# librosa/librosa

Measured on AMD Instinct MI355X. Metric: STFT+mel frames/sec (n_fft=2048 hop=512), higher is better.
Workload: dtype f32

## Files before the change

### librosa_amd/csrc/lra_fft.h

```cpp
#pragma once

#include <cmath>

#include "lra_common.h"

namespace lra {

template <int LOGM_, int LOGR_, class T_, int NTMIN_ = 256, int MINW_ = 0, bool HOIST_ = true, bool REV_ = false, int PLAN_ = 0> struct FftCfg {
    using real = T_;
    using cplx = cx<T_>;
    static constexpr int LOGM = LOGM_;
    static constexpr int M = 1 << LOGM_;
    static constexpr int N = 2 * M;
    static constexpr int LOGR = LOGR_ < LOGM_ ? LOGR_ : LOGM_;
    static constexpr int R = 1 << LOGR;
    static constexpr int TF = M / R;
    static constexpr int NT = TF > NTMIN_ ? TF : NTMIN_;
    static constexpr int FPB = NT / TF;
    static constexpr int P = (LOGM + LOGR - 1) / LOGR;
    static constexpr bool REV = REV_;
    static constexpr int PLAN = PLAN_;
    static constexpr int logr(int p) {
        if (PLAN_ == 1 && REV_) return p == 0 ? LOGM - (P - 1) * LOGR : LOGR;
        if (PLAN_ == 1) return (p + 1) * LOGR <= LOGM ? LOGR : LOGM - p * LOGR;
        return LOGM / P + ((REV_ ? p >= P - LOGM % P : p < LOGM % P) ? 1 : 0);
    }
    static constexpr int logs(int p) {
        int s = 0;
        for (int q = 0; q < p; ++q) s += logr(q);
        return s;
    }
    static constexpr int tw_off(int p) {
        int o = 0;
        for (int q = 1; q < p; ++q) o += ((1 << logr(q)) - 1) << logs(q);
        return o;
    }
    static constexpr int TW_TOTAL = tw_off(P) > 0 ? tw_off(P) : 1;
    static constexpr int treg_off(int p) {
        int o = 0;
        for (int q = 1; q < p; ++q) o += (R >> logr(q)) * logr(q);
        return o;
    }
    static constexpr int TREG_TOTAL = treg_off(P) > 0 ? treg_off(P) : 1;
    static constexpr int PADSHIFT = logr(0);
    static constexpr int FRAME_ELEMS = M + (M >> PADSHIFT) + 1;
    static constexpr int FRAME_BYTES = ((FRAME_ELEMS * (int)sizeof(cplx) + 15) / 16) * 16;
    static constexpr int phys(int i) { return i + (i >> PADSHIFT); }
    static constexpr int MIN_WAVES = MINW_ > 0 ? MINW_ : 2;
    static constexpr bool HOIST = HOIST_;
    template <int NT2> using with_nt = FftCfg<LOGM_, LOGR_, T_, NT2, MINW_, HOIST_, REV_, PLAN_>;
    static constexpr bool WAVE_SYNC = TF <= 64;
};

template <class T> LRA_HD cx<T> mul_w16(cx<T> a, int idx) {
    const T h = (T)0.70710678118654752440;
    const T c1 = (T)0.92387953251128675613, s1 = (T)0.38268343236508977173;
    switch (idx) {
        case 0: return a;
        case 4: return cmul_mi(a);
        case 2: return mk<T>((a.x + a.y) * h, (a.y - a.x) * h);
        case 6: return mk<T>((a.y - a.x) * h, -(a.x + a.y) * h);
        case 1: return mk<T>(a.x * c1 + a.y * s1, a.y * c1 - a.x * s1);
        case 3: return mk<T>(a.x * s1 + a.y * c1, a.y * s1 - a.x * c1);
        case 5: return mk<T>(a.y * c1 - a.x * s1, -(a.x * c1 + a.y * s1));
        default:  return mk<T>(a.y * s1 - a.x * c1, -(a.x * s1 + a.y * c1));
    }
}

template <int idx, class T> LRA_HD void bfly_w16(cx<T> e, cx<T> o, cx<T>& p, cx<T>& m) {
    const T h = (T)0.70710678118654752440;
    const T c1 = (T)0.92387953251128675613, s1 = (T)0.38268343236508977173;
    if constexpr (idx == 0) {
        p = cadd(e, o);
        m = csub(e, o);
    } else if constexpr (idx == 4) {
        p = add_mi(e, o);
        m = sub_mi(e, o);
    } else if constexpr (idx == 2) {
        const cx<T> u = add_mi(o, o);
        p = axpy(h, u, e);
        m = axpy(-h, u, e);
    } else if constexpr (idx == 6) {
        const cx<T> u = add_mi(o, o);
        p = axpy_mi(h, u, e);
        m = axpy_pi(h, u, e);
    } else if constexpr (idx == 1 || idx == 3) {
        const T c = idx == 1 ? c1 : s1, s = idx == 1 ? s1 : c1;
        p = axpy_mi(s, o, axpy(c, o, e));
        m = axpy_pi(s, o, axpy(-c, o, e));
    } else {
        const T c = idx == 5 ? c1 : s1, s = idx == 5 ? s1 : c1;
        p = axpy_mi(c, o, axpy(-s, o, e));
        m = axpy_pi(c, o, axpy(s, o, e));
    }
}

template <int r, class T> struct Dft {
    template <int k> static LRA_HD void stage(cx<T>* v, const cx<T>* e, const cx<T>* o) {
        if constexpr (k < r / 2) {
            bfly_w16<k * (16 / r), T>(e[k], o[k], v[k], v[k + r / 2]);
            stage<k + 1>(v, e, o);
        }
    }
    static LRA_HD void run(cx<T>* v) {
        cx<T> e[r / 2], o[r / 2];
        LRA_UNROLL
        for (int k = 0; k < r / 2; ++k) { e[k] = v[2 * k]; o[k] = v[2 * k + 1]; }
        Dft<r / 2, T>::run(e);
        Dft<r / 2, T>::run(o);
        stage<0>(v, e, o);
    }
};
template <class T> struct Dft<1, T> {
    static LRA_HD void run(cx<T>*) {}
};
template <class T> struct Dft<2, T> {
    static LRA_HD void run(cx<T>* v) {
        const cx<T> a = v[0], b = v[1];
        v[0] = cadd(a, b);
        v[1] = csub(a, b);
    }
};

template <class Cfg> constexpr int pstride(int c) { return c + (c >> Cfg::PADSHIFT); }
template <class Cfg> constexpr bool affine_tf() { return Cfg::TF % (1 << Cfg::PADSHIFT) == 0; }

template <class Cfg, int p> LRA_HD void pass_read(typename Cfg::cplx* v, Lds fr, int tf) {
    using C = typename Cfg::cplx;
    constexpr int lr = Cfg::logr(p), r = 1 << lr, nb = Cfg::R >> lr, sin = Cfg::M >> lr, Q = 1 << Cfg::PADSHIFT;
    if constexpr (affine_tf<Cfg>() && sin % Q == 0) {
        const int base = Cfg::phys(tf) * (int)sizeof(C);
        LRA_UNROLL
        for (int i = 0; i < nb; ++i) {
            LRA_UNROLL
            for (int j = 0; j < r; ++j) v[i * r + j] = lds_ld<C>(fr, base + (i * pstride<Cfg>(Cfg::TF) + j * pstride<Cfg>(sin)) * (int)sizeof(C));
        }
    } else {
        LRA_UNROLL
        for (int i = 0; i < nb; ++i) {
            const int b = tf + i * Cfg::TF;
            LRA_UNROLL
            for (int j = 0; j < r; ++j) v[i * r + j] = lds_ld<C>(fr, Cfg::phys(b + j * sin) * (int)sizeof(C));
        }
    }
}

template <class Cfg, int p> LRA_HD void pass_twiddle_dft(typename Cfg::cplx* v, int tf, const typename Cfg::cplx* __restrict__ tw) {
    using T = typename Cfg::real;
    constexpr int lr = Cfg::logr(p), r = 1 << lr, nb = Cfg::R >> lr, s = 1 << Cfg::logs(p);
    LRA_UNROLL
    for (int i = 0; i < nb; ++i) {
        const int b = tf + i * Cfg::TF;
        if (p > 0) {
            const int k = b & (s - 1);
            typename Cfg::cplx q[r];
            LRA_UNROLL
            for (int j = 1; j < r; ++j) q[j] = cmul_p(v[i * r + j], tw[Cfg::tw_off(p) + (j - 1) * s + k]);
            LRA_UNROLL
            for (int j = 1; j < r; ++j) v[i * r + j] = cmul_f(v[i * r + j], tw[Cfg::tw_off(p) + (j - 1) * s + k], q[j]);
        }
        Dft<r, T>::run(v + i * r);
    }
}

constexpr int popcount_c(int j) { int c = 0; for (; j; j >>= 1) c += j & 1; return c; }
constexpr int msb_c(int j) { int m = 0; for (int t = 0; t < 16; ++t) if ((j >> t) & 1) m = t; return m; }

template <class Cfg, int p> LRA_HD void pass_twiddle_dft_reg(typename Cfg::cplx* v, const typename Cfg::cplx* treg) {
    using T = typename Cfg::real;
    using C = typename Cfg::cplx;
    constexpr int lr = Cfg::logr(p), r = 1 << lr, nb = Cfg::R >> lr;
    LRA_UNROLL
    for (int i = 0; i < nb; ++i) {
        if (p > 0) {
            C w[r], q[r];
            LRA_UNROLL
            for (int j = 1; j < r; ++j)
                if (popcount_c(j) == 1) w[j] = treg[Cfg::treg_off(p) + i * lr + msb_c(j)];
            LRA_UNROLL
            for (int level = 2; level <= lr; ++level) {
                LRA_UNROLL
                for (int j = 1; j < r; ++j)
                    if (popcount_c(j) == level) q[j] = cmul_p(w[j - (1 << msb_c(j))], treg[Cfg::treg_off(p) + i * lr + msb_c(j)]);
                LRA_UNROLL
                for (int j = 1; j < r; ++j)
                    if (popcount_c(j) == level) w[j] = cmul_f(w[j - (1 << msb_c(j))], treg[Cfg::treg_off(p) + i * lr + msb_c(j)], q[j]);
            }
            LRA_UNROLL
            for (int j = 1; j < r; ++j) q[j] = cmul_p(v[i * r + j], w[j]);
            LRA_UNROLL
            for (int j = 1; j < r; ++j) v[i * r + j] = cmul_f(v[i * r + j], w[j], q[j]);
        }
        Dft<r, T>::run(v + i * r);
    }
}

template <class Cfg, int p> LRA_HD void load_pass_twiddles(typename Cfg::cplx* treg, int tf, const typename Cfg::cplx* __restrict__ tw) {
    constexpr int lr = Cfg::logr(p), nb = Cfg::R >> lr, s = 1 << Cfg::logs(p);
    LRA_UNROLL
    for (int i = 0; i < nb; ++i) {
        const int k = (tf + i * Cfg::TF) & (s - 1);
        LRA_UNROLL
        for (int t = 0; t < lr; ++t) treg[Cfg::treg_off(p) + i * lr + t] = tw[Cfg::tw_off(p) + ((1 << t) - 1) * s + k];
    }
}

template <class Cfg, int p> LRA_HD void pass_write(const typename Cfg::cplx* v, Lds fr, int tf) {
    using C = typename Cfg::cplx;
    constexpr int lr = Cfg::logr(p), r = 1 << lr, nb = Cfg::R >> lr, s = 1 << Cfg::logs(p);
    constexpr bool last = p == Cfg::P - 1;
    if constexpr (affine_tf<Cfg>() && p == 0) {
        const int base = tf * (r + 1) * (int)sizeof(C);
        LRA_UNROLL
        for (int i = 0; i < nb; ++i) {
            LRA_UNROLL
            for (int j = 0; j < r; ++j) lds_st<C>(fr, base + (i * Cfg::TF * (r + 1) + j) * (int)sizeof(C), v[i * r + j]);
        }
    } else if constexpr (affine_tf<Cfg>() && p > 0 && (last || Cfg::TF % s == 0)) {
        int base;
        if (last) {
            base = Cfg::phys(tf) * (int)sizeof(C);
        } else {
            const int k = tf & (s - 1);
            base = Cfg::phys(((tf - k) << lr) + k) * (int)sizeof(C);
        }
        constexpr int istep = last ? pstride<Cfg>(Cfg::TF) : pstride<Cfg>(Cfg::TF << lr);
        LRA_UNROLL
        for (int i = 0; i < nb; ++i) {
            LRA_UNROLL
            for (int j = 0; j < r; ++j) lds_st<C>(fr, base + (i * istep + j * pstride<Cfg>(s)) * (int)sizeof(C), v[i * r + j]);
        }
    } else {
        LRA_UNROLL
        for (int i = 0; i < nb; ++i) {
            const int b = tf + i * Cfg::TF;
            const int k = b & (s - 1);
            const int base = ((b - k) << lr) + k;
            LRA_UNROLL
            for (int j = 0; j < r; ++j) lds_st<C>(fr, Cfg::phys(base + j * s) * (int)sizeof(C), v[i * r + j]);
        }
    }
}

template <class Cfg> LRA_HD int last_pass_pos(int tf, int i, int j) {
    constexpr int p = Cfg::P - 1, s = 1 << Cfg::logs(p);
    return (tf + i * Cfg::TF) + j * s;
}

template <class Cfg> inline void build_pass_twiddles(typename Cfg::cplx* out) {
    const double two_pi = 6.283185307179586476925286766559;
    for (int p = 1; p < Cfg::P; ++p) {
        const int r = 1 << Cfg::logr(p), s = 1 << Cfg::logs(p);
        for (int j = 1; j < r; ++j)
            for (int k = 0; k < s; ++k) {
                const double ang = -two_pi * (double)k * (double)j / ((double)s * (double)r);
                out[Cfg::tw_off(p) + (j - 1) * s + k] = mk<typename Cfg::real>((typename Cfg::real)std::cos(ang), (typename Cfg::real)std::sin(ang));
            }
    }
}
template <class Cfg> constexpr int split_tw_count() { return Cfg::M + 1; }
template <class Cfg> inline void build_split_twiddles(typename Cfg::cplx* out) {
    const double two_pi = 6.283185307179586476925286766559;
    for (int k = 0; k <= Cfg::M; ++k) {
        const double ang = -two_pi * (double)k / (double)Cfg::N;
        out[k] = mk<typename Cfg::real>((typename Cfg::real)std::cos(ang), (typename Cfg::real)std::sin(ang));
    }
}

}
```

### librosa_amd/csrc/lra_kernels2.h

```cpp
#pragma once

#include "lra_kernels.h"

namespace lra {

template <class Cfg> constexpr bool v2_cfg_ok() {
    constexpr int pl = Cfg::P - 1;
    return Cfg::P >= 2 && Cfg::R == 16 && Cfg::HOIST && sizeof(typename Cfg::real) == 4 && affine_tf<Cfg>() && (Cfg::R >> Cfg::logr(pl)) == 2 &&
           2 * Cfg::TF == (Cfg::M >> Cfg::logr(pl)) && (Cfg::M >> Cfg::logr(pl)) % (1 << Cfg::PADSHIFT) == 0;
}
template <class Cfg> constexpr bool v2_hd_ok(int hd) { return (hd == 1 || hd == 2 || hd == 4 || hd == 8) && (1 << Cfg::logr(0)) % hd == 0; }
template <class Cfg> LRA_HD int v2_hop_divisor(int hop) {
    for (int hd = 1; hd <= 8; hd *= 2)
        if (hop * hd == Cfg::N && v2_hd_ok<Cfg>(hd)) return hd;
    return 0;
}

constexpr int kV2PrioA = 3, kV2PrioS = 2, kV2PrioB = 0, kV2PrioB3 = 1;
constexpr int kV2PrioCA = 3, kV2PrioCS = 2;
constexpr int kV2PrioPA = 3, kV2PrioPS = 2;
template <int P> LRA_HD void v2_setprio() { lra_setprio<P>(); }

template <class Cfg, int HD> struct Regs2 {
    using C = typename Cfg::cplx;
// ... 55 lines not shown
    using RG = Regs2<Cfg, HD>;
    if (next >= a.n_frames) return;
    const T* __restrict__ yb = a.y + (long long)clip * a.y_stride;
    const long long p0 = (long long)next * a.hop;
    const long long g0 = p0 + (Cfg::N - a.hop) - a.pad;
    if (LRA_LIKELY(g0 >= 0 && g0 + a.hop <= a.n)) {
        const T* __restrict__ src = yb + (p0 - a.pad) + 2 * tf;
        if (LRA_LIKELY((reinterpret_cast<size_t>(src) & (2 * sizeof(T) - 1)) == 0)) {
            LRA_UNROLL
            for (int n = 0; n < RG::NEW; ++n) {
                const int e = RG::elem_of_new(n);
                rg.pf[n] = *reinterpret_cast<const C*>(src + 2 * ((e / RG::r0) * Cfg::TF + (e % RG::r0) * RG::sin0));
            }
        } else {
            LRA_UNROLL
            for (int n = 0; n < RG::NEW; ++n) {
                const int e = RG::elem_of_new(n);
                const T* __restrict__ s2 = src + 2 * ((e / RG::r0) * Cfg::TF + (e % RG::r0) * RG::sin0);
                rg.pf[n] = mk<T>(s2[0], s2[1]);
            }
        }
    } else {
        LRA_UNROLL
        for (int n = 0; n < RG::NEW; ++n) {
            const long long p = p0 + 2 * RG::q_of(tf, RG::elem_of_new(n));
            rg.pf[n] = mk<T>(fetch_sample<T>(yb, p, a.pad, a.n, a.pad_mode), fetch_sample<T>(yb, p + 1, a.pad, a.n, a.pad_mode));
        }
    }
}

template <class Cfg, int HD> LRA_HD void v2_fill(const StftArgs<typename Cfg::real>& a, int clip, int frame, int tf, Regs2<Cfg, HD>& rg) {
    using T = typename Cfg::real;
    using RG = Regs2<Cfg, HD>;
    const T* __restrict__ yb = a.y + (long long)clip * a.y_stride;
    const long long p0 = (long long)frame * a.hop;
    LRA_UNROLL
    for (int e = 0; e < Cfg::R; ++e) {
        const long long p = p0 + 2 * RG::q_of(tf, e);
        const bool live = frame < a.n_frames;
        rg.raw[e] = live ? mk<T>(fetch_sample<T>(yb, p, a.pad, a.n, a.pad_mode), fetch_sample<T>(yb, p + 1, a.pad, a.n, a.pad_mode)) : mk<T>((T)0, (T)0);
    }
}

template <class Cfg, int HD> LRA_HD void v2_shift(Regs2<Cfg, HD>& rg) {
    using RG = Regs2<Cfg, HD>;
    LRA_UNROLL
    for (int i = 0; i < RG::nb0; ++i) {
        LRA_UNROLL
        for (int j = 0; j < RG::r0; ++j) rg.raw[i * RG::r0 + j] = j + RG::SJ < RG::r0 ? rg.raw[i * RG::r0 + j + RG::SJ] : rg.pf[i * RG::SJ + (j + RG::SJ - RG::r0)];
    }
}

template <class Cfg, int HD> LRA_HD void v2_window_rotating_ref(int it, Regs2<Cfg, HD>& rg) {
    using T = typename Cfg::real;
    using RG = Regs2<Cfg, HD>;
    constexpr int r0 = RG::r0, nb0 = RG::nb0, SJ = RG::SJ;
    const int rot = it & (HD - 1);
    for (int i = 0; i < nb0; ++i) {
        if (it > 0)
            for (int m = 0; m < SJ; ++m) rg.raw[i * r0 + (SJ * ((rot + HD - 1) % HD) + m) % r0] = rg.pf[i * SJ + m];
        for (int j = 0; j < r0; ++j) {
            const typename Cfg::cplx x = rg.raw[i * r0 + (j + SJ * rot) % r0], w = rg.win2[i * r0 + j];
            rg.v[i * r0 + j] = mk<T>(x.x * w.x, x.y * w.y);
        }
    }
}
template <class Cfg, int HD> constexpr bool v2_rotate_asm_ok() {
    return HD == 4 && Regs2<Cfg, HD>::r0 == 16 && Regs2<Cfg, HD>::nb0 == 1 && sizeof(typename Cfg::real) == 4;
}
#if defined(LRA_PK_ASM)
__device__ __forceinline__ void v2_rot_class(pk::f2& p0, pk::f2& p1, pk::f2& p2, pk::f2& p3, pk::f2 pf, pk::f2 w0, pk::f2 w1, pk::f2 w2, pk::f2 w3, pk::f2& v0, pk::f2& v1,
                                              pk::f2& v2, pk::f2& v3, int rot, int ins) {
    asm("s_cmp_lg_u32 %13, 0\n\t"
        "s_cbranch_scc1 .Lrot1_%=\n\t"
        "s_cmp_eq_u32 %14, 0\n\t"
        "s_cbranch_scc1 .Lrot0_%=\n\t"
        "v_mov_b64 %7, %8\n"
        ".Lrot0_%=:\n\t"
        "v_pk_mul_f32 %0, %4, %9\n\t"
        "v_pk_mul_f32 %1, %5, %10\n\t"
        "v_pk_mul_f32 %2, %6, %11\n\t"
        "v_pk_mul_f32 %3, %7, %12\n\t"
        "s_branch .Lrotend_%=\n"
        ".Lrot1_%=:\n\t"
        "s_cmp_lg_u32 %13, 1\n\t"
        "s_cbranch_scc1 .Lrot2_%=\n\t"
        "v_pk_mul_f32 %0, %5, %9\n\t"
        "v_pk_mul_f32 %1, %6, %10\n\t"
        "v_pk_mul_f32 %2, %7, %11\n\t"
        "v_pk_mul_f32 %3, %8, %12\n\t"
        "v_mov_b64 %4, %8\n\t"
        "s_branch .Lrotend_%=\n"
        ".Lrot2_%=:\n\t"
        "s_cmp_lg_u32 %13, 2\n\t"
        "s_cbranch_scc1 .Lrot3_%=\n\t"
        "v_pk_mul_f32 %0, %6, %9\n\t"
        "v_pk_mul_f32 %1, %7, %10\n\t"
        "v_pk_mul_f32 %2, %4, %11\n\t"
        "v_pk_mul_f32 %3, %8, %12\n\t"
        "v_mov_b64 %5, %8\n\t"
        "s_branch .Lrotend_%=\n"
        ".Lrot3_%=:\n\t"
        "v_pk_mul_f32 %0, %7, %9\n\t"
        "v_pk_mul_f32 %1, %4, %10\n\t"
        "v_pk_mul_f32 %2, %5, %11\n\t"
        "v_pk_mul_f32 %3, %8, %12\n\t"
        "v_mov_b64 %6, %8\n"
        ".Lrotend_%=:\n\t"
        "s_nop 0"
        : "=&v"(v0), "=&v"(v1), "=&v"(v2), "=&v"(v3), "+v"(p0), "+v"(p1), "+v"(p2), "+v"(p3)
        : "v"(pf), "v"(w0), "v"(w1), "v"(w2), "v"(w3), "s"(rot), "s"(ins)
        : "scc");
}
#endif
template <class Cfg, int HD> LRA_HD void v2_window_rotating(int it, Regs2<Cfg, HD>& rg) {
#if defined(LRA_PK_ASM)
    if constexpr (v2_rotate_asm_ok<Cfg, HD>()) {
        const int rot = it & 3, ins = it;
        pk::f2 p[16], o[16];
        LRA_UNROLL
        for (int e = 0; e < 16; ++e) p[e] = pk::v(rg.raw[e]);
        LRA_UNROLL
        for (int c = 0; c < 4; ++c)
            v2_rot_class(p[c], p[c + 4], p[c + 8], p[c + 12], pk::v(rg.pf[c]), pk::v(rg.win2[c]), pk::v(rg.win2[c + 4]), pk::v(rg.win2[c + 8]), pk::v(rg.win2[c + 12]), o[c],
                         o[c + 4], o[c + 8], o[c + 12], rot, ins);
        LRA_UNROLL
        for (int e = 0; e < 16; ++e) { rg.raw[e] = pk::c(p[e]); rg.v[e] = pk::c(o[e]); }
        return;
    }
#endif
    v2_window_rotating_ref<Cfg, HD>(it, rg);
}
template <class Cfg, int HD> LRA_HD void v2_pass0_dft(int tf, Regs2<Cfg, HD>& rg, Lds fr) {
    using T = typename Cfg::real;
    constexpr int r0 = Regs2<Cfg, HD>::r0, nb0 = Regs2<Cfg, HD>::nb0;
    LRA_UNROLL
    for (int i = 0; i < nb0; ++i) Dft<r0, T>::run(rg.v + i * r0);
    pass_write<Cfg, 0>(rg.v, fr, tf);
}

template <class Cfg, int HD> LRA_HD void v2_pass0(bool live, int tf, Regs2<Cfg, HD>& rg, Lds fr) {
    using T = typename Cfg::real;
    constexpr int r0 = Regs2<Cfg, HD>::r0, nb0 = Regs2<Cfg, HD>::nb0;
    (void)live;
    LRA_UNROLL
    for (int e = 0; e < Cfg::R; ++e) rg.v[e] = mk<T>(rg.raw[e].x * rg.win2[e].x, rg.raw[e].y * rg.win2[e].y);
    LRA_UNROLL
    for (int i = 0; i < nb0; ++i) Dft<r0, T>::run(rg.v + i * r0);
    pass_write<Cfg, 0>(rg.v, fr, tf);
}

template <class Cfg, int HD> LRA_HD void v2_last_read(Regs2<Cfg, HD>& rg, Lds fr, int tf) {
    using C = typename Cfg::cplx;
    constexpr int p = Cfg::P - 1, lr = Cfg::logr(p), r = 1 << lr, sin = Cfg::M >> lr;
    const int bA = Cfg::phys(tf) * (int)sizeof(C);
    const int bB = Cfg::phys(v2_mirror_bfly<Cfg>(tf)) * (int)sizeof(C);
    LRA_UNROLL
    for (int j = 0; j < r; ++j) {
        rg.v[j] = lds_ld<C>(fr, bA + j * pstride<Cfg>(sin) * (int)sizeof(C));
        rg.v[r + j] = lds_ld<C>(fr, bB + j * pstride<Cfg>(sin) * (int)sizeof(C));
    }
}


template <class T> struct alignas(16) V4 {
    T a, b, c, d;
};
template <class Cfg> constexpr bool v2_pw_swz() { return (2 * Cfg::TF) % 128 == 0; }
template <bool SWZ> LRA_HD int v2_pw_index_t(int k) {
    if (SWZ) return (k >> 3) * 8 + ((((k >> 2) ^ (k >> 7)) & 1) << 2) + (k & 3);
    return (k >> 3) * 12 + (k & 7);
}
template <class Cfg> LRA_HD int v2_pw_index(int k) { return v2_pw_index_t<v2_pw_swz<Cfg>()>(k); }
template <class Cfg> constexpr int v2_pw_bytes() { return (v2_pw_swz<Cfg>() ? Cfg::M + 8 : (Cfg::M >> 3) * 12 + 4) * (int)sizeof(typename Cfg::real); }

template <class Cfg> LRA_HD void v2_pw_addr_xor(Lds stage, int tf, int tfh, bool l0, int (&ak)[2][2], int (&am)[2][2]) {
    using T = typename Cfg::real;
    constexpr int p = Cfg::P - 1, r = 1 << Cfg::logr(p), s = 2 * Cfg::TF, M = Cfg::M, SZ = (int)sizeof(T);
    static_assert(v2_pw_swz<Cfg>() && SZ == 4 && s == 128, "bit 4 of the byte address swaps the halves of a run, bit 7 of the bin selects");
    constexpr int LOW = M - (r - 1) * s;
    ak[0][0] = lds_addr(stage, tf * SZ);
    ak[1][0] = lds_addr(stage, tfh * SZ);
    am[1][1] = lds_addr(stage, (LOW - tfh) * SZ);
    LRA_UNROLL
    for (int f = 0; f < 2; ++f) ak[f][1] = ak[f][0] ^ 16;
    am[1][0] = am[1][1] ^ 16;
    am[0][0] = l0 ? lds_addr(stage, LOW * SZ) : am[1][0];
    am[0][1] = am[0][0] ^ 16;
}

template <class Cfg, int HD, int MODE, int PM, bool PIN = true>
LRA_HD void v2_last_split_store(const StftArgs<typename Cfg::real>& a, int clip, int frame, bool valid, int tf, Regs2<Cfg, HD>& rg, Lds stage) {
    using T = typename Cfg::real;
    using C = typename Cfg::cplx;
    constexpr int p = Cfg::P - 1, r = 1 << Cfg::logr(p), s = 2 * Cfg::TF, M = Cfg::M;
    static_assert(r * s == M, "last pass: r butterfly outputs s apart");
    pass_twiddle_dft_reg<Cfg, p>(rg.v, rg.treg);
    const C* A = rg.v;
    const C* B = rg.v + r;
    const bool l0 = tf == 0;
    const LaneMask l0m = lane_mask(l0);
    const int tfh = v2_tf_hi<Cfg>(tf);
    const long long row = ((long long)clip * a.n_frames + frame) * a.row_pitch;
    C* __restrict__ const D = MODE == OUT_COMPLEX ? a.D + row : nullptr;
    T* __restrict__ const S = MODE == OUT_POWER ? a.S + row : nullptr;
    int pwk[2][2] = {{0, 0}, {0, 0}}, pwm[2][2] = {{0, 0}, {0, 0}};
    constexpr bool AXOR = MODE == OUT_MELR && !PIN && v2_pw_swz<Cfg>();
    constexpr bool POW2 = MODE == OUT_MELR && PM == POW_TWO;
    int ak[2][2] = {{0, 0}, {0, 0}}, am[2][2] = {{0, 0}, {0, 0}};
    if constexpr (AXOR) v2_pw_addr_xor<Cfg>(stage, tf, tfh, l0, ak, am);
    if (MODE == OUT_MELR && !AXOR) {
        LRA_UNROLL
        for (int par = 0; par < 2; ++par) {
            pwk[0][par] = v2_pw_index<Cfg>(tf + par * s) * (int)sizeof(T);
            pwk[1][par] = v2_pw_index<Cfg>(tfh + par * s) * (int)sizeof(T);
            pwm[0][par] = v2_pw_index<Cfg>(M - tf - par * s) * (int)sizeof(T);
            pwm[1][par] = v2_pw_index<Cfg>(M - tfh - par * s) * (int)sizeof(T);
            if (PIN) { LRA_KEEP(pwk[0][par]); LRA_KEEP(pwk[1][par]); LRA_KEEP(pwm[0][par]); LRA_KEEP(pwm[1][par]); }
        }
    }
    LRA_UNROLL
    for (int q = 0; q < r; ++q) {
        const C zk = q >= r / 2 ? sel_mask(l0m, l0, B[q - r / 2], A[q]) : A[q];
        C zm;
        if (q == 0) zm = B[r - 1];
        else if (q < r / 2) zm = sel_mask(l0m, l0, A[r - q], B[r - 1 - q]);
        else zm = sel_mask(l0m, l0, B[3 * r / 2 - 1 - q], B[r - 1 - q]);
        C xk = mk<T>((T)0, (T)0), xm = xk;
        C pp = xk;
        if constexpr (POW2) pp = split_pair_pow2<T>(zk, zm, rg.twr[q]);
        else split_pair<T>(zk, zm, rg.twr[q], xk, xm);
        if (q == 0) {
            const C z0 = A[0];
            const C dc = mk<T>((T)2 * (z0.x + z0.y), (T)0), ny = mk<T>((T)2 * (z0.x - z0.y), (T)0);
            if constexpr (POW2) {
                pp = mk<T>(sel_mask(l0m, l0, dc.x * dc.x, pp.x), sel_mask(l0m, l0, ny.x * ny.x, pp.y));
            } else {
                xk = sel_mask(l0m, l0, dc, xk);
                xm = sel_mask(l0m, l0, ny, xm);
            }
            if (LRA_UNLIKELY(l0 && valid && a.nonfinite_flag && !(std::fabs(dc.x) <= std::numeric_limits<T>::max()))) LRA_ATOMIC_OR(a.nonfinite_flag, 1u);
        }
        const int k = (q < r / 2 ? tf : tfh) + q * s;
        if (MODE == OUT_MELR) {
            const T vk = POW2 ? pp.x : spec_power<T, PM>(xk, a.power), vm = POW2 ? pp.y : spec_power<T, PM>(xm, a.power);
            if constexpr (AXOR) {
                lds_st_addr<T>(stage, ak[q < r / 2 ? 0 : 1][q & 1] + ((q & 1) * s + (q >> 1) * 2 * s) * (int)sizeof(T), vk);
                lds_st_addr<T>(stage, am[q < r / 2 ? 0 : 1][q & 1] + ((1 - (q & 1)) * s + (r / 2 - 1 - (q >> 1)) * 2 * s) * (int)sizeof(T), vm);
            } else if (v2_pw_swz<Cfg>()) {
                lds_st<T>(stage, pwk[q < r / 2 ? 0 : 1][q & 1] + (q >> 1) * 2 * s * (int)sizeof(T), vk);
                lds_st<T>(stage, pwm[q < r / 2 ? 0 : 1][q & 1] - (q >> 1) * 2 * s * (int)sizeof(T), vm);
            } else {
                lds_st<T>(stage, pwk[q < r / 2 ? 0 : 1][0] + 24 * q * (s / 16) * (int)sizeof(T), vk);
                lds_st<T>(stage, pwm[q < r / 2 ? 0 : 1][0] - 24 * q * (s / 16) * (int)sizeof(T), vm);
            }
        } else if (MODE == OUT_COMPLEX) {
            if (valid) { stream_store(&D[k], xk); stream_store(&D[M - k], xm); }
        } else {
            const T pk = spec_power<T, PM>(xk, a.power), pm = spec_power<T, PM>(xm, a.power);
            if (valid) { S[k] = pk; S[M - k] = pm; }
        }
    }
    const C zmid = A[r / 2];
    const C xmid = mk<T>((T)2 * zmid.x, (T)-2 * zmid.y);
    if (MODE == OUT_MELR) {
        if (l0) lds_st<T>(stage, v2_pw_index<Cfg>(M / 2) * (int)sizeof(T), spec_power<T, PM>(xmid, a.power));
    } else if (l0 && valid) {
        if (MODE == OUT_COMPLEX) D[M / 2] = xmid;
        else S[M / 2] = spec_power<T, PM>(xmid, a.power);
    }
}


template <class Cfg, int HD> LRA_HD void v2_mel_runs_read(Regs2<Cfg, HD>& rg, Lds pwr, int tf) {
    using T = typename Cfg::real;
    constexpr int BPL = Cfg::R / 2;
    static_assert(BPL == 8, "runs of 8 bins");
    LRA_UNROLL
    for (int run = 0; run < 2; ++run) {
        const int first = 8 * (run * Cfg::TF + tf);
        const V4<T> lo = lds_ld<V4<T>>(pwr, v2_pw_index<Cfg>(first) * (int)sizeof(T)), hi = lds_ld<V4<T>>(pwr, v2_pw_index<Cfg>(first + 4) * (int)sizeof(T));
        T* d = rg.pw + run * BPL;
        d[0] = lo.a; d[1] = lo.b; d[2] = lo.c; d[3] = lo.d; d[4] = hi.a; d[5] = hi.b; d[6] = hi.c; d[7] = hi.d;
    }
    rg.pw_extra = lds_ld<T>(pwr, (tf == 0 ? v2_pw_index<Cfg>(Cfg::M) : 0) * (int)sizeof(T));
}

template <class Cfg, int HD> LRA_HD void v2_mel_weights_read(Regs2<Cfg, HD>& rg, Lds sh, int tf) {
    using T = typename Cfg::real;
    constexpr int BPL = Cfg::R / 2, TF = Cfg::TF;
    LRA_UNROLL
    for (int run = 0; run < 2; ++run) {
        LRA_UNROLL
        for (int j = 0; j < BPL; j += 2) {
            const V4<T> w2 = lds_ld<V4<T>>(sh, ((BPL + 2) * (run * TF + tf) + j) * 2 * (int)sizeof(T));
            rg.v[run * BPL + j] = mk<T>(w2.a, w2.b);
            rg.v[run * BPL + j + 1] = mk<T>(w2.c, w2.d);
        }
    }
}

template <class Cfg, int HD> LRA_HD void v2_mel_accumulate(const StftArgs<typename Cfg::real>& a, int tf, Regs2<Cfg, HD>& rg, Lds rs, Lds sh) {
    using T = typename Cfg::real;
    using C = typename Cfg::cplx;
    constexpr int BPL = Cfg::R / 2, TF = Cfg::TF;
    const C* w = rg.v;
    LRA_UNROLL
    for (int run = 0; run < 2; ++run) {
        C acc = mk<T>((T)0, (T)0);
        LRA_UNROLL
        for (int j = 0; j < BPL; ++j) {
            const int jj = run * BPL + j;
            const T p = rg.pw[jj], keep = rg.keep[jj];
// ... 331 lines not shown
```

### librosa_amd/csrc/lra_kernels_pc.h

```cpp
#pragma once

#include "lra_kernels2.h"

namespace lra {

constexpr int kPcPrioPA = 3, kPcPrioPS = 2, kPcPrioCA = 0, kPcPrioCB = 1;
constexpr int kPcSpinLimit = 1 << 22;

template <class Cfg> struct PcLayout {
    using T = typename Cfg::real;
    static constexpr int NP = 2;
    static constexpr int NT = (NP + 1) * Cfg::TF;
    static constexpr int FRAME = Cfg::FRAME_BYTES;
    static constexpr int PW = (v2_pw_bytes<Cfg>() + 15) / 16 * 16;
    static constexpr int RS = ((Cfg::R * (Cfg::TF + kMelRsPitchExtra) + 2) * 2 * (int)sizeof(T) + 15) / 16 * 16;
    static constexpr int frame_off(int s) { return s * FRAME; }
    static constexpr int pw_off(int s) { return NP * FRAME + s * PW; }
    static constexpr int rs_off() { return NP * (FRAME + PW); }
    static constexpr int flags_off() { return rs_off() + RS; }
    static constexpr int ready_off(int s) { return flags_off() + 4 * s; }
    static constexpr int consumed_off(int s) { return flags_off() + 4 * (NP + s); }
    static constexpr int BYTES = flags_off() + 16;
};

// ... 23 lines not shown
    C w[Cfg::R];
    C wq;
    T keep[Cfg::R];
    T pw[Cfg::R], pw_extra;
    int mad[NB][2 * PH];
    int pwa[4], pwx;
    T* row[NB];
    int ph[NP][NB];
    PcTileV mt[NP];
};
template <class Cfg> LRA_HD bool pc_tile_uniform(const StftArgs<typename Cfg::real>& a) { return (a.n_frames & 3) == 0 && Cfg::TF >= 64; }
#ifdef LRA_HOSTSIM
LRA_HD int pc_mad_addr(Lds wg, int ad) { return ad; }
LRA_HD cx<float> pc_pair_ld(Lds wg, int addr) { return lds_ld<cx<float>>(wg, addr); }
#else
__device__ __forceinline__ int pc_mad_addr(Lds wg, int ad) {
    int addr = (int)(unsigned int)(size_t)(__attribute__((address_space(3))) char*)(wg.base + ad);
    asm volatile("" : "+v"(addr));
    return addr;
}
__device__ __forceinline__ cx<float> pc_pair_ld(Lds, int addr) {
    typedef float f2v __attribute__((ext_vector_type(2)));
    const f2v t = *(const volatile __attribute__((address_space(3))) f2v*)(size_t)(unsigned int)addr;
    return __builtin_bit_cast(cx<float>, t);
}
#endif
template <class T, int MT> LRA_HD void pc_tile_band(const PcTileV& t, int b, T (&out)[MT]) {
    LRA_UNROLL
    for (int k = 0; k < MT; ++k) out[k] = t[MT * b + k];
}

#ifdef LRA_HOSTSIM
LRA_HD int pc_flag_load(Lds l, int off) { return lds_ld<int>(l, off); }
LRA_HD void pc_flag_store(Lds l, int off, int v) { lds_st<int>(l, off, v); }
LRA_HD void pc_wait(Lds, int, int, unsigned int*) {}
LRA_HD void pc_fence() {}
#else
__device__ __forceinline__ void pc_fence() {
    __builtin_amdgcn_fence(__ATOMIC_RELEASE, "wavefront");
    __builtin_amdgcn_wave_barrier();
    __builtin_amdgcn_fence(__ATOMIC_ACQUIRE, "wavefront");
}
__device__ __forceinline__ int pc_flag_load(Lds l, int off) { return *(const volatile __attribute__((address_space(3))) int*)(l.base + off); }
__device__ __forceinline__ void pc_flag_store(Lds l, int off, int v) { *(volatile __attribute__((address_space(3))) int*)(l.base + off) = v; }
__device__ __forceinline__ void pc_wait(Lds l, int off, int want, unsigned int* sticky) {
    int spins = 0;
    while (true) {
        const int v = LRA_UNIFORM(pc_flag_load(l, off));
        if (LRA_LIKELY(v >= want)) break;
        if (LRA_UNLIKELY(++spins > kPcSpinLimit)) {
            if (sticky && (threadIdx.x & 63) == 0) atomicOr(sticky, 2u);
            break;
        }
        __builtin_amdgcn_s_sleep(2);
    }
    pc_fence();
}
__device__ __forceinline__ void pc_wait_ready(Lds l, int off, int want, unsigned int* sticky) {
    if (LRA_UNLIKELY(LRA_UNIFORM(pc_flag_load(l, off)) < want)) pc_wait(l, off, want, sticky);
    else pc_fence();
}
#endif

template <class Cfg, int HD> LRA_HD void pc_producer_prologue(const StftArgs<typename Cfg::real>& a, int clip, int frame0, int tf, Regs2<Cfg, HD>& rg) {
    using T = typename Cfg::real;
    if constexpr (Cfg::PLAN == 1) v3_hoist<Cfg, HD>(rg, tf, a.win, a.tw, a.twr);
    else v2_hoist<Cfg, HD>(rg, tf, a.win, a.tw, a.twr);
    v2_fill<Cfg, HD>(a, clip, frame0, tf, rg);
    if constexpr (v2_rotate_asm_ok<Cfg, HD>()) {
        LRA_UNROLL
        for (int e = 0; e < Cfg::R; ++e) { LRA_KEEP(rg.raw[e].x); LRA_KEEP(rg.raw[e].y); }
    }
    LRA_UNROLL
    for (int e = 0; e < Regs2<Cfg, HD>::NEW; ++e) rg.pf[e] = mk<T>((T)0, (T)0);
}
template <class Cfg, int HD> LRA_HD void pc_producer_pass0(const StftArgs<typename Cfg::real>& a, int clip, int frame, int it, bool more, int tf, Regs2<Cfg, HD>& rg, Lds fr) {
    if (v2_rotate_asm_ok<Cfg, HD>()) {
        v2_window_rotating<Cfg, HD>(it, rg);
        if (more) v2_issue_loads<Cfg, HD>(a, clip, frame + 1, tf, rg);
        v2_pass0_dft<Cfg, HD>(tf, rg, fr);
    } else {
        if (it > 0) v2_shift<Cfg, HD>(rg);
        if (more) v2_issue_loads<Cfg, HD>(a, clip, frame + 1, tf, rg);
        v2_pass0<Cfg, HD>(frame < a.n_frames, tf, rg, fr);
    }
}

template <class Cfg, int p> LRA_HD void pc_mid_dft_write(typename Cfg::cplx* v, const typename Cfg::cplx* treg, Lds fr, int tf) {
    if constexpr (Cfg::PLAN == 1) {
        v3_mid_twiddle_dft<Cfg>(v, treg);
        v3_mid_write<Cfg>(v, fr, tf);
    } else {
        pass_twiddle_dft_reg<Cfg, p>(v, treg);
        pass_write<Cfg, p>(v, fr, tf);
    }
}
template <class Cfg, int HD> LRA_HD void pc_last_read(Regs2<Cfg, HD>& rg, Lds fr, int tf) {
    if constexpr (Cfg::PLAN == 1) v3_last_read<Cfg, HD>(rg, fr, tf);
    else v2_last_read<Cfg, HD>(rg, fr, tf);
}
template <class Cfg, int HD, int PM> LRA_HD void pc_last_power_row(const StftArgs<typename Cfg::real>& a, int clip, int frame, int tf, Regs2<Cfg, HD>& rg, Lds pwr) {
    if constexpr (Cfg::PLAN == 1) v3_last_split_store<Cfg, HD, OUT_MELR, PM, false>(a, clip, frame, frame < a.n_frames, tf, rg, pwr);
    else v2_last_split_store<Cfg, HD, OUT_MELR, PM, false>(a, clip, frame, frame < a.n_frames, tf, rg, pwr);
}

template <class Cfg> LRA_HD void pc_consumer_prologue(const StftArgs<typename Cfg::real>& a, int clip, int f_first, int iters, int tf, PcRegs<Cfg>& rg, Lds wg) {
    using T = typename Cfg::real;
    using C = typename Cfg::cplx;
    using RG = PcRegs<Cfg>;
    constexpr int BPL = Cfg::R / 2, TF = Cfg::TF;
    const C* __restrict__ w2 = reinterpret_cast<const C*>(a.melr_w);
    LRA_UNROLL
    for (int run = 0; run < 2; ++run) {
        LRA_UNROLL
        for (int j = 0; j < BPL; ++j) rg.w[run * BPL + j] = w2[BPL * (run * TF + tf) + j];
    }
    rg.wq = w2[Cfg::M];
    LRA_UNROLL
    for (int jj = 0; jj < Cfg::R; ++jj) rg.keep[jj] = a.melr_keep[jj * TF + tf];
    LRA_UNROLL
    for (int b = 0; b < RG::NB; ++b) {
        const int m = RG::NB * tf + b;
        LRA_UNROLL
        for (int h = 0; h < 2; ++h) {
            LRA_UNROLL
            for (int q = 0; q < RG::PH; ++q) {
                const int ad = PcLayout<Cfg>::rs_off() + (m < a.n_mels ? a.melr_addr[(h * a.melr_pmax + q) * a.n_mels + m] : a.melr_zero);
                rg.mad[b][h * RG::PH + q] = pc_mad_addr(wg, ad & ~(2 * (int)sizeof(T) - 1));
            }
        }
    }
    LRA_UNROLL
    for (int run = 0; run < 2; ++run) {
        const int first = 8 * (run * TF + tf);
        rg.pwa[2 * run] = v2_pw_index<Cfg>(first) * (int)sizeof(T);
        rg.pwa[2 * run + 1] = v2_pw_index<Cfg>(first + 4) * (int)sizeof(T);
    }
    rg.pwx = (tf == 0 ? v2_pw_index<Cfg>(Cfg::M) : 0) * (int)sizeof(T);
    LRA_UNROLL
    for (int b = 0; b < RG::NB; ++b) {
        const int m = RG::NB * tf + b;
        rg.row[b] = a.Mel + ((long long)clip * a.n_mels + (m < a.n_mels ? m : 0)) * a.n_frames;
    }
    LRA_UNROLL
    for (int s = 0; s < RG::NP; ++s) {
        LRA_UNROLL
        for (int b = 0; b < RG::NB; ++b) {
            rg.ph[s][b] = (int)(((long long)clip * a.n_mels * a.n_frames + (long long)b * a.n_frames + f_first + s * iters) & (RG::TILE - 1));
            LRA_UNROLL
            for (int k = 0; k < RG::TILE; ++k) rg.mt[s][RG::TILE * b + k] = (T)0;
        }
    }
    rg.pw_extra = (T)0;
}
template <class Cfg> LRA_HD void pc_runs_read(PcRegs<Cfg>& rg, Lds pwr) {
    using T = typename Cfg::real;
    constexpr int BPL = Cfg::R / 2;
    static_assert(BPL == 8, "runs of 8 bins");
    LRA_UNROLL
    for (int run = 0; run < 2; ++run) {
        const V4<T> lo = lds_ld<V4<T>>(pwr, rg.pwa[2 * run]), hi = lds_ld<V4<T>>(pwr, rg.pwa[2 * run + 1]);
        T* d = rg.pw + run * BPL;
        d[0] = lo.a; d[1] = lo.b; d[2] = lo.c; d[3] = lo.d; d[4] = hi.a; d[5] = hi.b; d[6] = hi.c; d[7] = hi.d;
    }
    rg.pw_extra = lds_ld<T>(pwr, rg.pwx);
}
template <class Cfg> LRA_HD void pc_accumulate(const StftArgs<typename Cfg::real>& a, int tf, PcRegs<Cfg>& rg, Lds rs) {
    using T = typename Cfg::real;
    using C = typename Cfg::cplx;
    constexpr int BPL = Cfg::R / 2, TF = Cfg::TF;
    LRA_UNROLL
    for (int run = 0; run < 2; ++run) {
        C acc = mk<T>((T)0, (T)0);
        LRA_UNROLL
        for (int j = 0; j < BPL; ++j) {
            const int jj = run * BPL + j;
            const T p = rg.pw[jj], keep = rg.keep[jj];
            acc = mk<T>(acc.x * keep + rg.w[jj].x * p, acc.y * keep + rg.w[jj].y * p);
            lds_st<C>(rs, (jj * mel_runs_pitch(TF, 1) + tf) * (int)sizeof(C), acc);
        }
    }
    if (tf == 0) {
        lds_st<C>(rs, a.melr_mid, mk<T>(rg.wq.x * rg.pw_extra, rg.wq.y * rg.pw_extra));
        lds_st<C>(rs, a.melr_zero, mk<T>((T)0, (T)0));
    }
}
template <class Cfg, int S, bool UNI> LRA_HD PcTileV pc_combine(const StftArgs<typename Cfg::real>& a, int clip, int frame, int tf, int it, bool last_of_slot, PcRegs<Cfg>& rg, Lds wg, PcTileV mt) {
    using T = typename Cfg::real;
    using RG = PcRegs<Cfg>;
    constexpr int PH = RG::PH, NB = RG::NB, MT = RG::TILE;
    T x[NB][2 * PH];
    LRA_UNROLL
    for (int b = 0; b < NB; ++b) {
        LRA_UNROLL
        for (int q = 0; q < 2 * PH; ++q) {
            const cx<T> pr = pc_pair_ld(wg, rg.mad[b][q]);
            x[b][q] = q < PH ? pr.y : pr.x;
        }
    }
    LRA_UNROLL
    for (int b = 0; b < NB; ++b) {
        const int m = NB * tf + b;
        if (m >= a.n_mels) break;
        T part[2];
        LRA_UNROLL
        for (int h = 0; h < 2; ++h) {
            T acc = (T)0;
            LRA_UNROLL
            for (int q = 0; q < PH; ++q) acc += x[b][h * PH + q];
            part[h] = acc;
        }
        const T v = part[0] + part[1];
        int s8;
        if constexpr (UNI) {
            s8 = (rg.ph[S][b] + it) & (MT - 1);
            mt[MT * b + s8] = v;
        } else {
            s8 = (int)((rg.row[b] - a.Mel + frame) & (MT - 1));
            LRA_UNROLL
            for (int k = 0; k < MT; ++k) mt[MT * b + k] = k == s8 ? v : mt[MT * b + k];
        }
        if (last_of_slot || s8 == MT - 1) {
            T t8[MT];
            pc_tile_band(mt, b, t8);
            melr_burst_row(rg.row[b] + (frame - s8), s8, it, t8);
        }
    }
    return mt;
}

#ifndef LRA_HOSTSIM
template <class Cfg, bool UNI> __device__ __forceinline__ void pc_consumer(const StftArgs<typename Cfg::real>& a, int clip, int f_first, int iters, int n_it, Lds lds) {
    using L = PcLayout<Cfg>;
    constexpr int TF = Cfg::TF;
    PcRegs<Cfg> rg;
    const Lds rs = lds_sub(lds, L::rs_off());
    const int tf = (int)(threadIdx.x & (TF - 1));
    pc_consumer_prologue<Cfg>(a, clip, f_first, iters, tf, rg, lds);
    pc_fence();
    for (int it = 0; it < n_it; ++it) {
#define LRA_PC_SERVE(S)                                                                                                        \
        {                                                                                                                      \
            const int frame = f_first + S * iters + it;                                                                       \
            v2_setprio<kPcPrioCA>();                                                                                      \
            pc_wait_ready(lds, L::ready_off(S), it + 1, a.nonfinite_flag);                                                     \
            pc_runs_read<Cfg>(rg, lds_sub(lds, L::pw_off(S)));                                                                 \
            pc_fence();                                                                                                        \
            if (tf == 0) pc_flag_store(lds, L::consumed_off(S), it + 1);                             \
            pc_fence();                                                                                                        \
            pc_accumulate<Cfg>(a, tf, rg, rs);                                                                                 \
            pc_fence();                                                                                                        \
            v2_setprio<kPcPrioCB>();                                                                                      \
            if (frame < a.n_frames) rg.mt[S] = pc_combine<Cfg, S, UNI>(a, clip, frame, tf, it, it + 1 == iters || frame + 1 >= a.n_frames, rg, lds, rg.mt[S]); \
            pc_fence();                                                                                                        \
        }
        LRA_PC_SERVE(0)
        LRA_PC_SERVE(1)
#undef LRA_PC_SERVE
    }
}
#endif

template <class Cfg, int HD, int PM = POW_TWO> LRA_HD void stft_pc_block(const StftArgs<typename Cfg::real>& a_in, const int blk, Lds lds) {
    static_assert(pc_cfg_ok<Cfg>(), "producer / consumer mel kernel: one wave per frame, mirrored last pass, swizzled power row");
    using T = typename Cfg::real;
    using L = PcLayout<Cfg>;
    using RG = Regs2<Cfg, HD>;
    constexpr int NP = L::NP, TF = Cfg::TF;
    StftArgs<T> a = a_in;
    const int clip = blk / a.wg_per_clip;
    const int f_first = (blk % a.wg_per_clip) * a.frames_per_wg;
    const int iters = a.frames_per_wg / NP;
    const int left = a.n_frames - f_first;
    const int n_it = left < iters ? left : iters;
#ifdef LRA_HOSTSIM
    LRA_REGS(RG, prg, L::NT);
    LRA_REGS(PcRegs<Cfg>, crg, L::NT);
    LRA_PHASE(L::NT, tid) {
        const int w = tid / TF, tf = tid % TF;
        if (w < NP) pc_producer_prologue<Cfg, HD>(a, clip, f_first + w * iters, tf, LRA_R(prg));
        else pc_consumer_prologue<Cfg>(a, clip, f_first, iters, tf, LRA_R(crg), lds);
        if (tid < 2 * NP) pc_flag_store(lds, L::flags_off() + 4 * tid, 0);
    } LRA_PHASE_END
    for (int it = 0; it < n_it; ++it) {
        LRA_PHASE(L::NT, tid) {
            const int w = tid / TF, tf = tid % TF;
            if (w < NP) pc_producer_pass0<Cfg, HD>(a, clip, f_first + w * iters + it, it, it + 1 < iters, tf, LRA_R(prg), lds_sub(lds, L::frame_off(w)));
        } LRA_PHASE_END_SYNC(true)
#define LRA_PC_MID(p)                                                                                                                   \
        if (Cfg::P - 1 > p) {                                                                                                           \
            LRA_PHASE(L::NT, tid) {                                                                                                     \
                if (tid / TF < NP) pass_read<Cfg, (p < Cfg::P ? p : 0)>(LRA_R(prg).v, lds_sub(lds, L::frame_off(tid / TF)), tid % TF);  \
            } LRA_PHASE_END_SYNC(true)                                                                                                  \
            LRA_PHASE(L::NT, tid) {                                                                                                     \
                if (tid / TF < NP) pc_mid_dft_write<Cfg, (p < Cfg::P ? p : 0)>(LRA_R(prg).v, LRA_R(prg).treg, lds_sub(lds, L::frame_off(tid / TF)), tid % TF); \
            } LRA_PHASE_END_SYNC(true)                                                                                                  \
        }
        LRA_PC_MID(1)
        LRA_PC_MID(2)
#undef LRA_PC_MID
        LRA_PHASE(L::NT, tid) {
            if (tid / TF < NP) pc_last_read<Cfg, HD>(LRA_R(prg), lds_sub(lds, L::frame_off(tid / TF)), tid % TF);
        } LRA_PHASE_END_SYNC(true)
        LRA_PHASE(L::NT, tid) {
            const int w = tid / TF, tf = tid % TF, frame = f_first + w * iters + it;
            if (w < NP) pc_last_power_row<Cfg, HD, PM>(a, clip, frame, tf, LRA_R(prg), lds_sub(lds, L::pw_off(w)));
        } LRA_PHASE_END
        for (int s = 0; s < NP; ++s) {
            LRA_PHASE(L::NT, tid) {
                if (tid / TF == NP) pc_runs_read<Cfg>(LRA_R(crg), lds_sub(lds, L::pw_off(s)));
            } LRA_PHASE_END_SYNC(true)
            LRA_PHASE(L::NT, tid) {
                if (tid / TF == NP) pc_accumulate<Cfg>(a, tid % TF, LRA_R(crg), lds_sub(lds, L::rs_off()));
            } LRA_PHASE_END_SYNC(true)
            LRA_PHASE(L::NT, tid) {
                const int tf = tid % TF, frame = f_first + s * iters + it;
                if (tid / TF == NP && frame < a.n_frames) {
                    const bool last = it + 1 == iters || frame + 1 >= a.n_frames;
                    if (pc_tile_uniform<Cfg>(a)) {
                        if (s == 0) LRA_R(crg).mt[0] = pc_combine<Cfg, 0, true>(a, clip, frame, tf, it, last, LRA_R(crg), lds, LRA_R(crg).mt[0]);
                        else LRA_R(crg).mt[1] = pc_combine<Cfg, 1, true>(a, clip, frame, tf, it, last, LRA_R(crg), lds, LRA_R(crg).mt[1]);
                    } else {
                        if (s == 0) LRA_R(crg).mt[0] = pc_combine<Cfg, 0, false>(a, clip, frame, tf, it, last, LRA_R(crg), lds, LRA_R(crg).mt[0]);
                        else LRA_R(crg).mt[1] = pc_combine<Cfg, 1, false>(a, clip, frame, tf, it, last, LRA_R(crg), lds, LRA_R(crg).mt[1]);
                    }
                }
            } LRA_PHASE_END_SYNC(true)
        }
        sim::state().barrier();
    }
#else
    static_assert((TF & (TF - 1)) == 0 && L::pw_off(0) % 32 == 0 && L::PW % 32 == 0, "lane mask; power rows start on 32 bytes (v2_pw_addr_xor)");
    if (threadIdx.x < 2 * NP) pc_flag_store(lds, L::flags_off() + 4 * (int)threadIdx.x, 0);
    phase_sync<false>();
    const int wave = LRA_UNIFORM((int)(threadIdx.x / TF));
    if (wave < NP) {
        RG rg;
        const Lds fr = lds_sub(lds, L::frame_off(wave)), pwr = lds_sub(lds, L::pw_off(wave));
// ... 49 lines not shown
```

Measured before the change: 643.1 million.

## Use bank-conflict-free LDS exchange layouts for the M=1024 radix-16 FFT passes

Adds alternative LDS exchange layouts for the n_fft=2048 configuration (TF=64, R=16). The first pass writes with a pitch-66 transposed layout, and the second-to-third pass exchange drops the padding. Reads and writes are generalised through base/offset helpers so the v2 last-pass read uses the same layout. The aim is fewer LDS bank conflicts and simpler address arithmetic in the pass exchanges. Separately, the per-frame zero store to melr_zero moves into one-time register initialisation, which removes a redundant LDS store per frame.

Result: faster. 654.8 million (median of 6 runs) (+1.8%).

```diff
diff --git a/librosa_amd/csrc/lra_fft.h b/librosa_amd/csrc/lra_fft.h
--- a/librosa_amd/csrc/lra_fft.h
+++ b/librosa_amd/csrc/lra_fft.h
@@ -46,6 +46,9 @@
     static constexpr int FRAME_ELEMS = M + (M >> PADSHIFT) + 1;
     static constexpr int FRAME_BYTES = ((FRAME_ELEMS * (int)sizeof(cplx) + 15) / 16) * 16;
     static constexpr int phys(int i) { return i + (i >> PADSHIFT); }
+    static constexpr bool X1T = TF == 64 && R == 16 && M == 1024 && logr(0) == 4 && sizeof(T_) == 4;
+    static constexpr bool X2U = X1T && PLAN_ == 0 && P == 3;
+    static constexpr int X1_PITCH = 66;
     static constexpr int MIN_WAVES = MINW_ > 0 ? MINW_ : 2;
     static constexpr bool HOIST = HOIST_;
     template <int NT2> using with_nt = FftCfg<LOGM_, LOGR_, T_, NT2, MINW_, HOIST_, REV_, PLAN_>;
@@ -125,15 +128,54 @@
 template <class Cfg> constexpr int pstride(int c) { return c + (c >> Cfg::PADSHIFT); }
 template <class Cfg> constexpr bool affine_tf() { return Cfg::TF % (1 << Cfg::PADSHIFT) == 0; }
 
+template <class Cfg, int p> constexpr bool xw_affine() {
+    constexpr int s = 1 << Cfg::logs(p);
+    return affine_tf<Cfg>() && (p == 0 || p == Cfg::P - 1 || Cfg::TF % s == 0);
+}
+template <class Cfg, int p> constexpr bool xr_affine() { return affine_tf<Cfg>() && (Cfg::M >> Cfg::logr(p)) % (1 << Cfg::PADSHIFT) == 0; }
+template <class Cfg, int p> constexpr int xw_layout() { return p == 0 && Cfg::X1T ? 1 : (p == 1 && Cfg::X2U ? 2 : 0); }
+template <class Cfg, int p> constexpr int xr_layout() { return p == 1 && Cfg::X1T ? 1 : (p == 2 && Cfg::X2U ? 2 : 0); }
+
+template <class Cfg, int p> LRA_HD constexpr int xw_base(int tf) {
+    constexpr int lr = Cfg::logr(p), r = 1 << lr, s = 1 << Cfg::logs(p);
+    if constexpr (p == 0) return xw_layout<Cfg, p>() == 1 ? tf : tf * (r + 1);
+    else if constexpr (p == Cfg::P - 1) return Cfg::phys(tf);
+    else {
+        const int k = tf & (s - 1);
+        const int e = ((tf - k) << lr) + k;
+        return xw_layout<Cfg, p>() == 2 ? e : Cfg::phys(e);
+    }
+}
+template <class Cfg, int p> constexpr int xw_off(int i, int j) {
+    constexpr int lr = Cfg::logr(p), r = 1 << lr, s = 1 << Cfg::logs(p);
+    if (p == 0) return xw_layout<Cfg, p>() == 1 ? Cfg::X1_PITCH * j : i * Cfg::TF * (r + 1) + j;
+    if (p == Cfg::P - 1) return i * pstride<Cfg>(Cfg::TF) + j * pstride<Cfg>(s);
+    return xw_layout<Cfg, p>() == 2 ? i * (Cfg::TF << lr) + j * s : i * pstride<Cfg>(Cfg::TF << lr) + j * pstride<Cfg>(s);
+}
+template <class Cfg, int p> LRA_HD constexpr int xr_base(int b) {
+    if constexpr (xr_layout<Cfg, p>() == 1) return Cfg::X1_PITCH * (b & 15) + (b >> 4);
+    else if constexpr (xr_layout<Cfg, p>() == 2) return b;
+    else return Cfg::phys(b);
+}
+template <class Cfg, int p> constexpr int xr_off(int i, int j) {
+    constexpr int sin = Cfg::M >> Cfg::logr(p);
+    if (xr_layout<Cfg, p>() == 1) return (i * Cfg::TF + j * sin) >> 4;
+    if (xr_layout<Cfg, p>() == 2) return i * Cfg::TF + j * sin;
+    return i * pstride<Cfg>(Cfg::TF) + j * pstride<Cfg>(sin);
+}
+template <class Cfg> constexpr int x_layout_units(int layout) { return layout == 1 ? Cfg::X1_PITCH * 15 + Cfg::TF : (layout == 2 ? Cfg::M : Cfg::phys(Cfg::M - 1) + 1); }
+
 template <class Cfg, int p> LRA_HD void pass_read(typename Cfg::cplx* v, Lds fr, int tf) {
     using C = typename Cfg::cplx;
-    constexpr int lr = Cfg::logr(p), r = 1 << lr, nb = Cfg::R >> lr, sin = Cfg::M >> lr, Q = 1 << Cfg::PADSHIFT;
-    if constexpr (affine_tf<Cfg>() && sin % Q == 0) {
-        const int base = Cfg::phys(tf) * (int)sizeof(C);
-        LRA_UNROLL
-        for (int i = 0; i < nb; ++i) {
-            LRA_UNROLL
-            for (int j = 0; j < r; ++j) v[i * r + j] = lds_ld<C>(fr, base + (i * pstride<Cfg>(Cfg::TF) + j * pstride<Cfg>(sin)) * (int)sizeof(C));
+    constexpr int lr = Cfg::logr(p), r = 1 << lr, nb = Cfg::R >> lr, sin = Cfg::M >> lr;
+    static_assert(xr_layout<Cfg, p>() == 0 || xr_affine<Cfg, p>(), "the exchange layouts have the affine form only");
+    static_assert(x_layout_units<Cfg>(xr_layout<Cfg, p>()) * (int)sizeof(C) <= Cfg::FRAME_BYTES, "exchange layout within the frame area");
+    if constexpr (xr_affine<Cfg, p>()) {
+        const int base = xr_base<Cfg, p>(tf) * (int)sizeof(C);
+        LRA_UNROLL
+        for (int i = 0; i < nb; ++i) {
+            LRA_UNROLL
+            for (int j = 0; j < r; ++j) v[i * r + j] = lds_ld<C>(fr, base + xr_off<Cfg, p>(i, j) * (int)sizeof(C));
         }
     } else {
         LRA_UNROLL
@@ -208,27 +250,13 @@
 template <class Cfg, int p> LRA_HD void pass_write(const typename Cfg::cplx* v, Lds fr, int tf) {
     using C = typename Cfg::cplx;
     constexpr int lr = Cfg::logr(p), r = 1 << lr, nb = Cfg::R >> lr, s = 1 << Cfg::logs(p);
-    constexpr bool last = p == Cfg::P - 1;
-    if constexpr (affine_tf<Cfg>() && p == 0) {
-        const int base = tf * (r + 1) * (int)sizeof(C);
-        LRA_UNROLL
-        for (int i = 0; i < nb; ++i) {
-            LRA_UNROLL
-            for (int j = 0; j < r; ++j) lds_st<C>(fr, base + (i * Cfg::TF * (r + 1) + j) * (int)sizeof(C), v[i * r + j]);
-        }
-    } else if constexpr (affine_tf<Cfg>() && p > 0 && (last || Cfg::TF % s == 0)) {
-        int base;
-        if (last) {
-            base = Cfg::phys(tf) * (int)sizeof(C);
-        } else {
-            const int k = tf & (s - 1);
-            base = Cfg::phys(((tf - k) << lr) + k) * (int)sizeof(C);
-        }
-        constexpr int istep = last ? pstride<Cfg>(Cfg::TF) : pstride<Cfg>(Cfg::TF << lr);
-        LRA_UNROLL
-        for (int i = 0; i < nb; ++i) {
-            LRA_UNROLL
-            for (int j = 0; j < r; ++j) lds_st<C>(fr, base + (i * istep + j * pstride<Cfg>(s)) * (int)sizeof(C), v[i * r + j]);
+    static_assert(xw_layout<Cfg, p>() == 0 || xw_affine<Cfg, p>(), "the exchange layouts have the affine form only");
+    if constexpr (xw_affine<Cfg, p>()) {
+        const int base = xw_base<Cfg, p>(tf) * (int)sizeof(C);
+        LRA_UNROLL
+        for (int i = 0; i < nb; ++i) {
+            LRA_UNROLL
+            for (int j = 0; j < r; ++j) lds_st<C>(fr, base + xw_off<Cfg, p>(i, j) * (int)sizeof(C), v[i * r + j]);
         }
     } else {
         LRA_UNROLL
diff --git a/librosa_amd/csrc/lra_kernels2.h b/librosa_amd/csrc/lra_kernels2.h
--- a/librosa_amd/csrc/lra_kernels2.h
+++ b/librosa_amd/csrc/lra_kernels2.h
@@ -231,13 +231,14 @@
 
 template <class Cfg, int HD> LRA_HD void v2_last_read(Regs2<Cfg, HD>& rg, Lds fr, int tf) {
     using C = typename Cfg::cplx;
-    constexpr int p = Cfg::P - 1, lr = Cfg::logr(p), r = 1 << lr, sin = Cfg::M >> lr;
-    const int bA = Cfg::phys(tf) * (int)sizeof(C);
-    const int bB = Cfg::phys(v2_mirror_bfly<Cfg>(tf)) * (int)sizeof(C);
+    constexpr int p = Cfg::P - 1, lr = Cfg::logr(p), r = 1 << lr;
+    static_assert(xr_affine<Cfg, p>(), "v2_cfg_ok: base + immediates (lra_fft.h, exchange addresses)");
+    const int bA = xr_base<Cfg, p>(tf) * (int)sizeof(C);
+    const int bB = xr_base<Cfg, p>(v2_mirror_bfly<Cfg>(tf)) * (int)sizeof(C);
     LRA_UNROLL
     for (int j = 0; j < r; ++j) {
-        rg.v[j] = lds_ld<C>(fr, bA + j * pstride<Cfg>(sin) * (int)sizeof(C));
-        rg.v[r + j] = lds_ld<C>(fr, bB + j * pstride<Cfg>(sin) * (int)sizeof(C));
+        rg.v[j] = lds_ld<C>(fr, bA + xr_off<Cfg, p>(0, j) * (int)sizeof(C));
+        rg.v[r + j] = lds_ld<C>(fr, bB + xr_off<Cfg, p>(0, j) * (int)sizeof(C));
     }
 }
 
diff --git a/librosa_amd/csrc/lra_kernels_pc.h b/librosa_amd/csrc/lra_kernels_pc.h
--- a/librosa_amd/csrc/lra_kernels_pc.h
+++ b/librosa_amd/csrc/lra_kernels_pc.h
@@ -199,6 +199,7 @@
         }
     }
     rg.pw_extra = (T)0;
+    if (tf == 0) lds_st<C>(lds_sub(wg, PcLayout<Cfg>::rs_off()), a.melr_zero, mk<T>((T)0, (T)0));
 }
 template <class Cfg> LRA_HD void pc_runs_read(PcRegs<Cfg>& rg, Lds pwr) {
     using T = typename Cfg::real;
@@ -227,10 +228,7 @@
             lds_st<C>(rs, (jj * mel_runs_pitch(TF, 1) + tf) * (int)sizeof(C), acc);
         }
     }
-    if (tf == 0) {
-        lds_st<C>(rs, a.melr_mid, mk<T>(rg.wq.x * rg.pw_extra, rg.wq.y * rg.pw_extra));
-        lds_st<C>(rs, a.melr_zero, mk<T>((T)0, (T)0));
-    }
+    if (tf == 0) lds_st<C>(rs, a.melr_mid, mk<T>(rg.wq.x * rg.pw_extra, rg.wq.y * rg.pw_extra));
 }
 template <class Cfg, int S, bool UNI> LRA_HD PcTileV pc_combine(const StftArgs<typename Cfg::real>& a, int clip, int frame, int tf, int it, bool last_of_slot, PcRegs<Cfg>& rg, Lds wg, PcTileV mt) {
     using T = typename Cfg::real;
```
